# real-stanford/flingbot

Hardware: AMD Instinct MI355X
Metric: sim steps/sec (64x64-particle cloth) (higher is better)
Workload: dtype f32

## Files before the change

flingbot_amd/csrc/fs_fused_grid_kernel.h:

```cpp
#pragma once
#include "fs_fused_kernel.h"

#define FG_PLANE (FS_FUSED_MAX_PARTICLES * 4)
#define FG_PAD 1024
#define FG_OFF_XX FG_PAD
#define FG_OFF_X0 (FG_OFF_XX + 4 * FG_PLANE)
#define FG_OFF_CACC (FG_OFF_X0 + 3 * FG_PLANE)
#define FG_OFF_CUR (FG_OFF_CACC + FS_FUSED_CSET_CAP * 16)
#define FG_OFF_ITEMS (FG_OFF_CUR + FS_FUSED_CUR_BYTES)
#define FG_OFF_SCAN (FG_OFF_ITEMS + FS_FUSED_MAX_PARTICLES * 2)
#define FG_OFF_CSET (FG_OFF_SCAN + 64)
#define FG_OFF_CHIST (FG_OFF_CSET + FS_FUSED_CSET_CAP * 2)
#define FG_OFF_ROWL (FG_OFF_CHIST + 512)
#define FG_OFF_KZ (FG_OFF_ROWL + 1024)
#define FG_OFF_KS (FG_OFF_KZ + 1024)
#define FG_OFF_COLL (FG_OFF_KS + 1024)
#define FG_OFF_RCNT (FG_OFF_COLL + 512)
#define FG_LDS_BYTES (FG_OFF_RCNT + 512)
static_assert(FG_OFF_ROWL % 8 == 0 && (FG_OFF_KZ - FG_OFF_ROWL) % 8 == 0, "row tables are read as ds_read_b64 pairs");
static_assert((FG_OFF_COLL - FG_OFF_KS) % 256 == 0, "column tables share one address, rows as ds_read2st64_b32 offsets");
static_assert(FG_LDS_BYTES <= 160 * 1024, "grid-64 kernel: the LDS of one CU");
static_assert(FG_OFF_CACC % 16 == 0 && FG_OFF_CUR == FG_OFF_CACC + FS_FUSED_CSET_CAP * 16, "set and queue accumulators: one array");
#ifndef FG_SINGLES
#define FG_SINGLES 1
// ... 12 lines not shown
    asm volatile("ds_read2st64_b32 %0, %1 offset0:%2 offset1:%3" : "=v"(x0) : "v"(a), "n"(DZ + 2), "n"(DZ + 3) : "memory");
    asm volatile("ds_read2st64_b32 %0, %1 offset0:%2 offset1:%3" : "=v"(x1) : "v"(a), "n"(DZ + 2 + 64), "n"(DZ + 3 + 64) : "memory");
    asm volatile("ds_read2st64_b32 %0, %1 offset0:%2 offset1:%3" : "=v"(x2) : "v"(a), "n"(DZ + 2 + 128), "n"(DZ + 3 + 128) : "memory");
}
template <int OFF>
__device__ __forceinline__ fs_f2 fg_load_rows(unsigned a) {
    static_assert(OFF >= 0 && OFF < 65536 && OFF % 8 == 0, "ds_read_b64 offset");
    fs_f2 r;
    asm volatile("ds_read_b64 %0, %1 offset:%2" : "=v"(r) : "v"(a), "n"(OFF) : "memory");
    return r;
}
template <int R0, int R1>
__device__ __forceinline__ fs_f2 fg_load_cols(unsigned a) {
    static_assert(R0 >= 0 && R0 < 256 && R1 >= 0 && R1 < 256, "ds_read2st64_b32 offsets");
    fs_f2 r;
    asm volatile("ds_read2st64_b32 %0, %1 offset0:%2 offset1:%3" : "=v"(r) : "v"(a), "n"(R0), "n"(R1) : "memory");
    return r;
}
#define FG_WAIT(N, A0, A1, A2) asm volatile("s_waitcnt lgkmcnt(" #N ")" : "+v"(A0), "+v"(A1), "+v"(A2))

#define FG_MIN_L2 1.17549435e-38f
__device__ __forceinline__ float fg_scale(float xi0, float xi1, float xi2, float xj0, float xj1, float xj2, float L, float k,
                                          float &l2) {
    const float ex = xi0 - xj0, ey = xi1 - xj1, ez = xi2 - xj2;
    l2 = fs_dot3(ex, ey, ez, ex, ey, ez);
    const float inv = __builtin_amdgcn_rsqf(l2);
    const float len = l2 * inv;
    const float C = len - L;
    return k * (C * inv);
}
__device__ __forceinline__ void fg_accum(float &d0, float &d1, float &d2, float xi0, float xi1, float xi2, float xj0, float xj1,
                                         float xj2, float sc) {
    const float ex = xi0 - xj0, ey = xi1 - xj1, ez = xi2 - xj2;
    d0 = FS_FMA(-ex, sc, d0);
    d1 = FS_FMA(-ey, sc, d1);
    d2 = FS_FMA(-ez, sc, d2);
}
__device__ __forceinline__ float fg_from_left(float v) {
    return __int_as_float(__builtin_amdgcn_update_dpp(0, __float_as_int(v), 0x138, 0xf, 0xf, true));
}
__device__ __forceinline__ float fg_from_right(float v) {
    return __int_as_float(__builtin_amdgcn_update_dpp(0, __float_as_int(v), 0x130, 0xf, 0xf, true));
}

__device__ __forceinline__ void fg_apply(const FsAcc &a, float relax, const float *rcnt, float &x0, float &x1, float &x2) {
    if (a.cnt > 0) {
        const float sc = a.cnt < 128 ? rcnt[a.cnt] : relax / (float)a.cnt;
        x0 = FS_FMA(a.d0, sc, x0); x1 = FS_FMA(a.d1, sc, x1); x2 = FS_FMA(a.d2, sc, x2);
    }
}

__global__ __launch_bounds__(FS_FUSED_THREADS) void fs_k_fused_grid64(const FsEnvDev *__restrict__ envs,
                                                                      const FsShapesDev *__restrict__ shapes, const int *ids,
                                                                      int n_steps) {
    static_assert(FS_FUSED_THREADS == 1024 && FS_FUSED_PPT == 4, "grid-64 kernel: 16 waves x 4 rows");
    extern __shared__ __attribute__((aligned(16))) char smem[];
    float *Xx = (float *)(smem + FG_OFF_XX);
    float *Xy = Xx + FS_FUSED_MAX_PARTICLES, *Xz = Xy + FS_FUSED_MAX_PARTICLES, *Xw = Xz + FS_FUSED_MAX_PARTICLES;
    float *X0x = (float *)(smem + FG_OFF_X0);
    float *X0y = X0x + FS_FUSED_MAX_PARTICLES;
    float *X0z = X0y + FS_FUSED_MAX_PARTICLES;
    unsigned short *cursor = (unsigned short *)(smem + FG_OFF_CUR);
    unsigned short *items = (unsigned short *)(smem + FG_OFF_ITEMS);
    int *wave_tot = (int *)(smem + FG_OFF_SCAN);
    float *rowL = (float *)(smem + FG_OFF_ROWL);

#ifdef FS_BLOCK_CLOCKS
    const unsigned long long tc_start = __builtin_amdgcn_s_memtime(), tr_start = __builtin_amdgcn_s_memrealtime();
#endif
#ifdef FS_TIMING
    unsigned long long ts_acc[16] = {0, 0, 0, 0, 0, 0, 0, 0, 0, 0, 0, 0, 0, 0, 0, 0};
    unsigned long long ts_last = __builtin_amdgcn_s_memtime();
#endif
    const int e = ids[blockIdx.x];
    if (e < 0) return;
    const FsEnvDev &E = envs[e];
    const FsShapesDev &sh = shapes[e];
    const FsFusedConsts c = fs_fused_consts(E, sh);
    const int n = c.n;
    const unsigned un = (unsigned)n;
    const int t = threadIdx.x, lane = t & 63, w = t >> 6;
    const int dimz = n >> 6;

    FsVec4 *const g_pos = E.pos, *const g_vel = E.vel;
    const FsVec4 *const g_rest = E.rest;
    const fs_gci g_phase = (fs_gci)E.phase;
    const fs_gi g_nlist = (fs_gi)E.nlist, g_ncount = (fs_gi)E.ncount;
    const fs_gci g_ell_j = (fs_gci)E.ell_j;
    const fs_gcf g_ell_len = (fs_gcf)E.ell_len, g_ell_k = (fs_gcf)E.ell_k;
    const fs_gcf g_L = (fs_gcf)E.g64_L;
    const int max_deg = E.max_deg;
    const fs_gcu g_near = (fs_gcu)E.restnear_w;

    int find_mode = 0;
    {
        const int ph0 = g_phase[0];
        int differs = 0;
        for (int i = t; i < n; i += FS_FUSED_THREADS) differs |= (g_phase[i] != ph0);
        if (t == 0) wave_tot[0] = 0;
        __syncthreads();
        if (differs) atomicOr(&wave_tot[0], 1);
        __syncthreads();
        const int mixed = wave_tot[0];
        __syncthreads();
        if (!mixed) {
            if (!(ph0 & FS_PHASE_SELF_COLLIDE)) find_mode = 3;
            else if (!(ph0 & FS_PHASE_SELF_COLLIDE_FILTER)) find_mode = 2;
            else if (E.restnear_ok == 2 && FS_STENCIL_FILTER) find_mode = 4;
            else if (E.restnear_ok) find_mode = 1;
        }
    }
    for (int q = t; q < FG_OFF_X0 / 4; q += FS_FUSED_THREADS) ((float *)smem)[q] = 0.0f;
    __syncthreads();
    for (int i = t; i < n; i += FS_FUSED_THREADS) {
        const FsVec4 p = fs_ld4(g_pos, i);
        Xx[i] = p.x; Xy[i] = p.y; Xz[i] = p.z; Xw[i] = p.w;
        X0x[i] = p.x; X0y[i] = p.y; X0z[i] = p.z;
    }
    if (t < 256) {
        const int r = t & 63, s = 8 + (t >> 6);
        rowL[t] = r < dimz ? g_L[(unsigned)s * un + (unsigned)(r * 64 + 2)] : 0.0f;
    }
    constexpr int XS_DX[4] = {-1, -2, +1, +2};
    constexpr int SH_DX[4] = {+1, -1, -1, +1}, SH_DZ[4] = {-1, -1, +1, +1};
    constexpr int ZS_DZ[4] = {-1, -2, +1, +2};
    float *colL = (float *)(smem + FG_OFF_COLL);
    if (t < 128) {
        const int col = t & 63, q = t >> 6;
        const int dxq = q == 0 ? -1 : -2;
        colL[t] = (unsigned)(col + dxq) < 64u ? g_L[(unsigned)q * un + (unsigned)(2 * 64 + col)] : 0.0f;
    }
    float *rcnt = (float *)(smem + FG_OFF_RCNT);
    if (t < 128) rcnt[t] = t > 0 ? c.relax / (float)t : 0.0f;
    if (t < 256) {
        const int c64 = t & 63, q = t >> 6;
        const int sdx = (q == 0 || q == 3) ? +1 : -1, sslot = q < 2 ? 2 + q : 4 + q;
        const int zdz = q < 2 ? -1 - q : q - 1;
        ((float *)(smem + FG_OFF_KS))[t] = (unsigned)(c64 + sdx) < 64u ? E.g64_kh[sslot] : 0.0f;
        ((float *)(smem + FG_OFF_KZ))[t] = (c64 < dimz && (unsigned)(c64 + zdz) < (unsigned)dimz) ? E.g64_kh[8 + q] : 0.0f;
    }
    const float kh0 = E.g64_kh[0], kh1 = E.g64_kh[1];
    unsigned nvalid = 0u;
#pragma unroll
    for (int k = 0; k < FS_FUSED_PPT; ++k) {
        const int row = FG_ROW(w, k);
        int cnt = 0;
#pragma unroll
        for (int q = 0; q < 4; ++q) {
            cnt += ((unsigned)(lane + XS_DX[q]) < 64u) ? 1 : 0;
            cnt += ((unsigned)(lane + SH_DX[q]) < 64u && (unsigned)(row + SH_DZ[q]) < (unsigned)dimz) ? 1 : 0;
            cnt += ((unsigned)(row + ZS_DZ[q]) < (unsigned)dimz) ? 1 : 0;
        }
        nvalid |= (unsigned)cnt << (8 * k);
    }
    __syncthreads();
    unsigned fastmask = 0u;
    {
        constexpr int cdx[FS_G64_SLOTS] = FS_G64_DX_LIST, cdz[FS_G64_SLOTS] = FS_G64_DZ_LIST;
#pragma unroll
        for (int k = 0; k < FS_FUSED_PPT; ++k) {
            const int row = FG_ROW(w, k), i = row * 64 + lane;
            bool differs = false;
            if (i < n) {
                const float wi = Xw[i];
                differs = !(wi > 0.0f);
#pragma unroll
                for (int q = 0; q < FS_G64_SLOTS; ++q) {
                    const bool in = (unsigned)(lane + cdx[q]) < 64u && (unsigned)(row + cdz[q]) < (unsigned)dimz;
                    if (in) differs |= Xw[i + cdz[q] * 64 + cdx[q]] != wi;
                }
            }
            if (i < n && __builtin_amdgcn_ballot_w64(differs) == 0ull) fastmask |= 1u << k;
        }
        fastmask = (unsigned)__builtin_amdgcn_readfirstlane((int)fastmask);
    }

    FS_TS(0)
#pragma unroll 1
    for (int frame = 0; frame < n_steps; ++frame) {
#pragma unroll 1
        for (int sub = 0; sub < c.substeps; ++sub) {
            for (int q = t; q < FS_FUSED_BUCKETS / 2; q += FS_FUSED_THREADS) ((unsigned *)cursor)[q] = 0u;
            FsVec4 xp[FS_FUSED_PPT];
#pragma unroll
            for (int k = 0; k < FS_FUSED_PPT; ++k) {
                const int i = t + k * FS_FUSED_THREADS;
                xp[k] = FsVec4{0.0f, 0.0f, 0.0f, 0.0f};
                if (i < n) {
                    const FsVec4 p0 = FsVec4{X0x[i], X0y[i], X0z[i], Xw[i]};
                    xp[k] = fs_fused_predict(c, p0, fs_ld4(g_vel, i));
                    fs_st4(E.x0, i, p0);
                }
            }
            __syncthreads();
            const fs_lu fill = (fs_lu)(smem + FG_OFF_XX + 2 * FG_PLANE);
            if (find_mode == 4)
                for (int q = t; q < FS_FUSED_MAX_PARTICLES; q += FS_FUSED_THREADS) fill[q] = 0u;
            fs_fused_build_grid(c, xp, cursor, items, wave_tot, X0x, X0y, X0z);
            FS_TS(1)
            const FsFindConsts fc = {n, c.ncap, c.rad2, c.inv_rad, find_mode, E.gp_dimx, E.gp_magic};
            if (find_mode == 4) {
                int *const any_over = wave_tot;
                if (t == 0) *any_over = 0;
                int sb0 = 0, sb1 = 0, sb2 = 0, sb3 = 0;
#pragma unroll 1
                for (int k = 0; k < FS_FUSED_PPT; ++k) {
                    const int qs = t + k * FS_FUSED_THREADS;
                    if (qs >= n) break;
                    const int i = items[qs];
                    const FsVec4 xi = FsVec4{X0x[qs], X0y[qs], X0z[qs], 0.0f};
                    const int shape_bits = (int)(fs_shape_candidates(E.p, sh, sub, xi.x, xi.y, xi.z) << FS_SHAPE_MASK_SHIFT);
                    if (k == 0) sb0 = shape_bits; else if (k == 1) sb1 = shape_bits; else if (k == 2) sb2 = shape_bits; else sb3 = shape_bits;
                    fs_pair_find_neighbors(fc, i, qs, xi, (fs_lcus)cursor, (fs_lcus)items, g_nlist, (fs_lus)(smem + FG_OFF_XX) + t,
                                           (fs_lcf)X0x, fill);
                }
                FS_TS(2)
                __syncthreads();
                FS_TS(3)
                unsigned overmask = 0u;
#pragma unroll 1
                for (int k = 0; k < FS_FUSED_PPT; ++k) {
                    const int qs = t + k * FS_FUSED_THREADS;
                    if (qs >= n) break;
                    const int i = items[qs];
                    const int cnt = (int)fill[i];
                    const int shape_bits = k == 0 ? sb0 : k == 1 ? sb1 : k == 2 ? sb2 : sb3;
                    if (cnt > c.ncap) {
                        overmask |= 1u << k;
                        continue;
                    }
                    fs_pair_sort_column(n, i, cnt, g_nlist);
                    g_ncount[i] = cnt | shape_bits;
                }
                if (overmask) atomicOr(any_over, 1);
                __syncthreads();
                if (*any_over) {
                    FsNearWords none;
#pragma unroll
                    for (int q = 0; q < 8; ++q) none.w[q] = 0xffffffffu;
#pragma unroll 1
                    for (int k = 0; k < FS_FUSED_PPT; ++k) {
                        if (!((overmask >> k) & 1u)) continue;
                        const int qs = t + k * FS_FUSED_THREADS;
                        const int i = items[qs];
                        const FsVec4 xi = FsVec4{X0x[qs], X0y[qs], X0z[qs], 0.0f};
                        const int shape_bits = k == 0 ? sb0 : k == 1 ? sb1 : k == 2 ? sb2 : sb3;
                        g_ncount[i] = fs_fused_find_neighbors<true>(fc, i, xi, (fs_lcus)cursor, (fs_lcus)items, g_phase, g_rest, g_nlist,
                                                                    none, (fs_lus)(smem + FG_OFF_XX) + t, (fs_lcf)X0x) | shape_bits;
                    }
                    __syncthreads();
                }
            } else {
#pragma unroll 1
                for (int qs = t; qs < n; qs += FS_FUSED_THREADS) {
                    const int i = items[qs];
                    const FsVec4 xi = FsVec4{X0x[qs], X0y[qs], X0z[qs], 0.0f};
                    const int shape_bits = (int)(fs_shape_candidates(E.p, sh, sub, xi.x, xi.y, xi.z) << FS_SHAPE_MASK_SHIFT);
                    FsNearWords near;
#pragma unroll
                    for (int q = 0; q < 8; ++q) near.w[q] = find_mode == 1 ? g_near[(unsigned)q * un + (unsigned)i] : 0xffffffffu;
                    g_ncount[i] = (find_mode == 3 ? 0
                                                  : fs_fused_find_neighbors<false>(fc, i, xi, (fs_lcus)cursor, (fs_lcus)items, g_phase,
                                                                                   g_rest, g_nlist, near,
                                                                                   (fs_lus)(smem + FG_OFF_XX) + t, (fs_lcf)X0x)) |
                                  shape_bits;
                }
                FS_TS(2)
                __syncthreads();
                FS_TS(3)
            }
#pragma unroll
            for (int k = 0; k < FS_FUSED_PPT; ++k) {
                const int i = t + k * FS_FUSED_THREADS;
                if (i < n) {
                    Xx[i] = xp[k].x; Xy[i] = xp[k].y; Xz[i] = xp[k].z; Xw[i] = xp[k].w;
                    const FsVec4 p0 = fs_ld4(E.x0, i);
                    X0x[i] = p0.x; X0y[i] = p0.y; X0z[i] = p0.z;
                } else {
                    Xx[i] = 0.0f; Xy[i] = 0.0f; Xz[i] = 0.0f; Xw[i] = 0.0f;
                }
            }

            unsigned short *cset = (unsigned short *)(smem + FG_OFF_CSET);
            FsVec4 *cacc = (FsVec4 *)(smem + FG_OFF_CACC);
            int *chist = (int *)(smem + FG_OFF_CHIST);
            if (t < 128) chist[t] = 0;
            int *nsingles = (int *)(smem + FG_OFF_SCAN);
            if (t == 0) *nsingles = 0;
            __syncthreads();
            int ccls[FS_FUSED_PPT];
#pragma unroll
            for (int k = 0; k < FS_FUSED_PPT; ++k) {
                const int i = FG_ROW(w, k) * 64 + lane;
                int cc = 0;
                if (i < n && Xw[i] > 0.0f) cc = g_ncount[i] & FS_NCOUNT_MASK;
                ccls[k] = cc > 96 ? 96 : cc;
                if (ccls[k] > 0) atomicAdd(&chist[ccls[k]], 1);
            }
            __syncthreads();
            fs_fused_count_offsets(chist, t);
            __syncthreads();
            FsVec4 *squeue = cacc + FS_FUSED_CSET_CAP;
            unsigned slotw[2] = {~0u, ~0u};
#pragma unroll
            for (int k = 0; k < FS_FUSED_PPT; ++k) {
                if (ccls[k] > 0) {
                    const int i = FG_ROW(w, k) * 64 + lane;
                    unsigned slot = FG_SLOT_INLINE;
                    const int pos = atomicAdd(&chist[ccls[k]], 1);
                    if (pos < FS_FUSED_CSET_CAP) {
                        cset[pos] = (unsigned short)i;
                        slot = (unsigned)pos;
                    }
#if FG_SINGLES
                    else if (ccls[k] <= 16) {
                        const int sp = atomicAdd(nsingles, 1);
                        if (sp < FG_SINGLES_CAP) {
                            slot = (unsigned)(FS_FUSED_CSET_CAP + sp);
                            squeue[sp].w = __int_as_float(i | (g_nlist[i] << 12) | ((ccls[k] - 1) << 28));
                        }
                    }
#endif
                    slotw[k >> 1] = (slotw[k >> 1] & ~(0xffffu << (16 * (k & 1)))) | (slot << (16 * (k & 1)));
                }
            }
            __syncthreads();
            const int csize = chist[0] < FS_FUSED_CSET_CAP ? chist[0] : FS_FUSED_CSET_CAP;
            const int n_singles = *nsingles < FG_SINGLES_CAP ? *nsingles : FG_SINGLES_CAP;
            const int i2 = t < csize ? (int)cset[t] : -1;
            int cnt2 = 0, cj2[FS_FUSED_PREFETCH_CAND];
#pragma unroll
            for (int q = 0; q < FS_FUSED_PREFETCH_CAND; ++q) cj2[q] = 0;
            if (i2 >= 0) {
                cnt2 = g_ncount[i2] & FS_NCOUNT_MASK;
#pragma unroll
                for (int q = 0; q < FS_FUSED_PREFETCH_CAND; ++q) cj2[q] = g_nlist[(unsigned)q * un + (unsigned)i2];
            }
            static_assert(FG_SINGLES_CAP <= 2 * FG_SINGLES_LANES, "two queue entries per lane");
            unsigned qw0 = 0u, qw1 = 0u;
#if FG_SINGLES
            if (t >= 64 && t - 64 < n_singles) qw0 = (unsigned)__float_as_int(squeue[t - 64].w);
            if (t >= 64 && t - 64 + FG_SINGLES_LANES < n_singles) qw1 = (unsigned)__float_as_int(squeue[t - 64 + FG_SINGLES_LANES].w);
            __syncthreads();
#endif

            FS_TS(4)
#pragma unroll 1
            for (int it = 0; it < c.iters; ++it) {
                unsigned cpack = 0u;
                float rold[2][3], rnew[2][3];
#pragma unroll
                for (int q = 0; q < 6; ++q) { rold[q / 3][q % 3] = 0.0f; rnew[q / 3][q % 3] = 0.0f; }
#ifdef FG_UNROLL_PAIRS
#pragma unroll
#else
#pragma unroll 1
#endif
                for (int pr = 0; pr < 2; ++pr) {
                    const int rowP = FG_ROW(w, 2 * pr);
                    const int iP_raw = rowP * 64 + lane, iQ_raw = iP_raw + 64;
                    const bool haveP = rowP < dimz, haveQ = rowP + 1 < dimz;
                    const int iP = haveP ? iP_raw : 0, iQ = haveQ ? iQ_raw : 0;
                    const bool fast = haveQ && ((fastmask >> (2 * pr)) & 3u) == 3u;
                    const fs_f2 xi0 = fs_f2{Xx[iP], Xx[iQ]}, xi1 = fs_f2{Xy[iP], Xy[iQ]}, xi2 = fs_f2{Xz[iP], Xz[iQ]};
                    const fs_f2 wi = fs_f2{Xw[iP], Xw[iQ]};
                    FsAcc aP, aQ;
                    bool exact = !fast;
                    if (fast) {
                        unsigned aLane = (unsigned)(lane * 4);
                        asm volatile("" : "+v"(aLane));
                        const unsigned am2 = (unsigned)(FG_OFF_XX + ((rowP - 2) * 64 - 2) * 4) + aLane;
                        const unsigned am1 = am2 + 4u, a00 = am2 + 8u, ap1 = am2 + 12u, ap2 = am2 + 16u;
                        constexpr int SH_SLOT[4] = {2, 3, 6, 7};
                        float sLP[2], sLQ[4];
#pragma unroll
                        for (int q = 0; q < 2; ++q) sLP[q] = g_L[(unsigned)SH_SLOT[q] * un + (unsigned)iP];
#pragma unroll
                        for (int q = 0; q < 4; ++q) sLQ[q] = g_L[(unsigned)SH_SLOT[q] * un + (unsigned)iQ];
                        const unsigned aRow = (unsigned)(FG_OFF_ROWL + rowP * 4), aCol = (unsigned)FG_OFF_KS + aLane;
                        constexpr int CL_ROW = (FG_OFF_COLL - FG_OFF_KS) / 256;
                        fs_f2 cL = fg_load_cols<CL_ROW, CL_ROW + 1>(aCol);
                        const unsigned aKP = rowP >= 1 ? aCol : aLane;
                        const unsigned aKQ = rowP + 2 < dimz ? aCol : aLane;
                        fs_f2 kP23 = fg_load_cols<0, 1>(aKP);
                        fs_f2 kQ23 = fg_load_cols<0, 1>(aCol);
#define FG_KX(q) ((unsigned)(lane + XS_DX[q]) < 64u ? (q == 0 ? kh0 : kh1) : 0.0f)
                        float dP0 = 0.0f, dP1 = 0.0f, dP2 = 0.0f, dQ0 = 0.0f, dQ1 = 0.0f, dQ2 = 0.0f, mP = 1.0f, mQ = 1.0f;
                        fs_f2 u0, u1, u2, v0, v1, v2;
                        float l2a, l2b, l2c, l2d;
                        fg_load_slot<0>(am1, u0, u1, u2);
                        fg_load_slot<0>(am2, v0, v1, v2);
                        asm volatile("s_waitcnt lgkmcnt(3)"
                                     : "+v"(cL), "+v"(kP23), "+v"(kQ23), "+v"(u0), "+v"(u1), "+v"(u2));
                        const float scP0 = fg_scale(xi0.x, xi1.x, xi2.x, u0.x, u1.x, u2.x, cL.x, FG_KX(0), l2a);
                        const float scQ0 = fg_scale(xi0.y, xi1.y, xi2.y, u0.y, u1.y, u2.y, cL.x, FG_KX(0), l2b);
                        fg_accum(dP0, dP1, dP2, xi0.x, xi1.x, xi2.x, u0.x, u1.x, u2.x, scP0);
                        fg_accum(dQ0, dQ1, dQ2, xi0.y, xi1.y, xi2.y, u0.y, u1.y, u2.y, scQ0);
                        __builtin_amdgcn_sched_barrier(0);
                        fg_load_slot<-1>(ap1, u0, u1, u2);
                        FG_WAIT(3, v0, v1, v2);
                        const float scP1 = fg_scale(xi0.x, xi1.x, xi2.x, v0.x, v1.x, v2.x, cL.y, FG_KX(1), l2c);
                        const float scQ1 = fg_scale(xi0.y, xi1.y, xi2.y, v0.y, v1.y, v2.y, cL.y, FG_KX(1), l2d);
                        fg_accum(dP0, dP1, dP2, xi0.x, xi1.x, xi2.x, v0.x, v1.x, v2.x, scP1);
                        fg_accum(dQ0, dQ1, dQ2, xi0.y, xi1.y, xi2.y, v0.y, v1.y, v2.y, scQ1);
                        mP = fminf(fminf(mP, l2a), l2c);
                        mQ = fminf(fminf(mQ, l2b), l2d);
                        __builtin_amdgcn_sched_barrier(0);
                        fg_load_slot<-1>(am1, v0, v1, v2);
// ... 191 lines not shown
                    int jn = more > 0 ? g_nlist[un + (unsigned)i] : 0;
                    const FsVec4 pa = squeue[q];
                    FsAcc a = {pa.x, pa.y, pa.z, __float_as_int(pa.w)};
                    const float xi0 = Xx[i], xi1 = Xy[i], xi2 = Xz[i], wi = Xw[i];
                    const float ri0 = xi0 - X0x[i], ri1 = xi1 - X0y[i], ri2 = xi2 - X0z[i];
#pragma unroll 1
                    for (int sq = 0; sq <= more; ++sq) {
                        const FsVec4 xj = FsVec4{Xx[j], Xy[j], Xz[j], Xw[j]};
                        fs_particle_contact(a, xi0, xi1, xi2, wi, ri0, ri1, ri2, xj, xj.x - X0x[j], xj.y - X0y[j], xj.z - X0z[j], c.restd,
                                            c.restd2, c.mu_p);
                        j = jn;
                        if (sq + 2 <= more) jn = g_nlist[(unsigned)(sq + 2) * un + (unsigned)i];
                    }
                    squeue[q] = FsVec4{a.d0, a.d1, a.d2, __int_as_float(a.cnt)};
                }
#endif
                FS_TS(8)
                __syncthreads();
                FS_TS(9)
#pragma unroll 1
                for (int pr = 0; pr < 2; ++pr) {
                    const int iP = FG_ROW(w, 2 * pr) * 64 + lane;
                    const unsigned slw = pr == 0 ? slotw[0] : slotw[1];
                    FsAcc a[2];
                    unsigned sm[2];
                    bool act[2];
                    float x0[2], x1[2], x2[2], r0[2], r1[2], r2[2];
                    int n_planes = c.n_planes, n_shapes = c.n_shapes;
                    asm volatile("" : "+s"(n_planes), "+s"(n_shapes));
#pragma unroll
                    for (int h = 0; h < 2; ++h) {
                        const int i = iP + 64 * h;
                        const unsigned myslot = h == 0 ? (slw & 0xffffu) : (slw >> 16);
                        act[h] = (i < n) & (Xw[i] > 0.0f);
                        a[h] = FsAcc{rold[h][0], rold[h][1], rold[h][2], (int)(h == 0 ? cpack >> 24 : (cpack >> 16) & 0xffu)};
                        if (act[h] && myslot < FG_SLOT_INLINE) {
                            const FsVec4 pa = cacc[myslot];
                            a[h] = FsAcc{pa.x, pa.y, pa.z, __float_as_int(pa.w)};
                        }
                        sm[h] = act[h] ? (pr == 0 ? smk[h] : smk[2 + h]) : 0u;
                        x0[h] = Xx[i]; x1[h] = Xy[i]; x2[h] = Xz[i];
                        r0[h] = x0[h] - X0x[i]; r1[h] = x1[h] - X0y[i]; r2[h] = x2[h] - X0z[i];
                    }
#pragma unroll
                    for (int q = 0; q < 3; ++q) { rold[0][q] = rnew[0][q]; rold[1][q] = rnew[1][q]; }
                    cpack <<= 16;
#pragma unroll
                    for (int h = 0; h < 2; ++h) {
                        int q = 0;
                        if (n_planes == 1) {
                            if (sm[h] & 1u)
                                fs_plane_contact(a[h], x0[h], x1[h], x2[h], r0[h], r1[h], r2[h], c.pl0, c.pl1, c.pl2, c.pl3, c.cd, c.mu_s,
                                                 c.mu_k);
                            q = 1;
                        }
                        for (; q < n_planes; ++q)
                            if ((sm[h] >> q) & 1u)
                                fs_plane_contact(a[h], x0[h], x1[h], x2[h], r0[h], r1[h], r2[h], E.p.planes[q][0], E.p.planes[q][1],
                                                 E.p.planes[q][2], E.p.planes[q][3], c.cd, c.mu_s, c.mu_k);
                    }
                    if (n_shapes != 0 && __builtin_amdgcn_ballot_w64(((sm[0] | sm[1]) >> FS_SHAPE_SPHERE_BIT) != 0u) != 0ull) {
                        const float S = (float)c.substeps;
#pragma unroll
                        for (int h = 0; h < 2; ++h)
                            for (int q = 0; q < n_shapes; ++q)
                                if ((sm[h] >> (FS_SHAPE_SPHERE_BIT + q)) & 1u) {
                                    float c0, c1, c2, s0, s1, s2;
                                    fs_shape_sweep(sh, q, sub, S, c0, c1, c2, s0, s1, s2);
                                    fs_sphere_contact(a[h], x0[h], x1[h], x2[h], r0[h], r1[h], r2[h], c0, c1, c2, sh.pos[q].w, s0, s1, s2,
                                                      c.cd, c.mu_s, c.mu_k);
                                }
                    }
#pragma unroll
                    for (int h = 0; h < 2; ++h)
                        if (act[h]) {
                            const int i = iP + 64 * h;
                            fg_apply(a[h], c.relax, rcnt, x0[h], x1[h], x2[h]);
                            Xx[i] = x0[h]; Xy[i] = x1[h]; Xz[i] = x2[h];
                        }
                }
                __syncthreads();
                FS_TS(10)
            }
            for (int i = t; i < n; i += FS_FUSED_THREADS) {
                const FsVec4 xf = FsVec4{Xx[i], Xy[i], Xz[i], Xw[i]};
                FsVec4 p0 = FsVec4{X0x[i], X0y[i], X0z[i], xf.w};
                FsVec4 v = fs_ld4(g_vel, i);
                fs_fused_finalize(c, p0, v, xf);
                fs_st4(g_vel, i, v);
                X0x[i] = p0.x; X0y[i] = p0.y; X0z[i] = p0.z;
            }
        }
    }
    for (int i = t; i < n; i += FS_FUSED_THREADS) fs_st4(g_pos, i, FsVec4{X0x[i], X0y[i], X0z[i], Xw[i]});
#ifdef FS_BLOCK_CLOCKS
    if (t == 0) {
        const unsigned long long tc_total = __builtin_amdgcn_s_memtime() - tc_start, tr_end = __builtin_amdgcn_s_memrealtime();
        const fs_gi out = g_nlist + 95u * un;
        out[0] = (int)(unsigned)tc_total; out[1] = (int)(unsigned)(tc_total >> 32);
        out[2] = (int)(unsigned)tr_start; out[3] = (int)(unsigned)tr_end;
    }
#endif
#ifdef FS_TIMING
    FS_TS(11)
#ifdef FS_TIMING_COUNTS
    if (blockIdx.x == 0 && t == 0)
        printf("DBG runs(wave) %llu trips(wave) %llu candidates(lane) %llu survivors(lane) %llu accepted(lane) %llu phaseB trips(wave) %llu\n",
               fs_dbg_cnt[0], fs_dbg_cnt[1], fs_dbg_cnt[2], fs_dbg_cnt[3], fs_dbg_cnt[4], fs_dbg_cnt[5]);
#endif
    if (blockIdx.x == 0 && (t & 63) == 0)
        printf("TS wave %2d: init %llu grid %llu find %llu findwait %llu cset %llu springs %llu park %llu bar1 %llu contact %llu bar2 %llu finish+bar3 %llu final %llu\n",
               t >> 6, ts_acc[0], ts_acc[1], ts_acc[2], ts_acc[3], ts_acc[4], ts_acc[5], ts_acc[6], ts_acc[7], ts_acc[8], ts_acc[9], ts_acc[10],
               ts_acc[11]);
#endif
}
```

flingbot_amd/csrc/fs_fused_kernel.h:

```cpp
#pragma once
#include "fs_constraints.h"
#include "fs_pair_search.h"

#ifndef FS_FUSED_THREADS
#define FS_FUSED_THREADS 1024
#endif
#define FS_FUSED_PPT (4096 / FS_FUSED_THREADS)
#define FS_FUSED_MAX_PARTICLES (FS_FUSED_THREADS * FS_FUSED_PPT)
#define FS_FUSED_MAX_DEG 64
#ifndef FS_STENCIL_FILTER
#define FS_STENCIL_FILTER 1
#endif
#ifndef FS_FUSED_BUCKET_BITS
#define FS_FUSED_BUCKET_BITS 13
#endif
#define FS_FUSED_BUCKETS (1 << FS_FUSED_BUCKET_BITS)
#define FS_FUSED_CUR_BYTES (FS_FUSED_BUCKETS * 2)
#define FS_FUSED_SLOTS 16

#define FS_FUSED_OFF_DICT 0
#define FS_FUSED_OFF_X (FS_FUSED_OFF_DICT + 256 * 8)
#define FS_FUSED_OFF_X0 (FS_FUSED_OFF_X + FS_FUSED_MAX_PARTICLES * 16)
#define FS_FUSED_OFF_CUR (FS_FUSED_OFF_X0 + FS_FUSED_MAX_PARTICLES * 12)
#define FS_FUSED_OFF_ITEMS (FS_FUSED_OFF_CUR + FS_FUSED_CUR_BYTES)
// ... 39 lines not shown
__device__ __forceinline__ void fs_st4o(FsVec4 *base, unsigned idx, const FsVec4 v) {
    *(FS_GLOBAL fs_f4 *)((FS_GLOBAL char *)base + (idx << 4)) = fs_f4{v.x, v.y, v.z, v.w};
}
template <typename T>
__device__ __forceinline__ T fs_ldo(const T *base, unsigned idx) {
    return *(FS_GLOBAL const T *)((FS_GLOBAL const char *)base + (idx << 2));
}

__device__ __forceinline__ int fs_fused_row(int cy, int cz) {
    return fs_pair_row(cy, cz, FS_FUSED_BUCKET_BITS);
}
__device__ __forceinline__ int fs_fused_bucket(int cx, int cy, int cz) {
    return (fs_fused_row(cy, cz) + cx) & (FS_FUSED_BUCKETS - 1);
}

struct FsFusedConsts {
    int n, substeps, iters, ncap, n_shapes, n_planes;
    float h, inv_h, g0, g1, g2, damping;
    float rad2, inv_rad, restd, restd2, mu_p, mu_s, mu_k, cd, relax, maxdv2, maxdv, thr2, max_speed;
    float pl0, pl1, pl2, pl3;
};

__device__ __forceinline__ FsFusedConsts fs_fused_consts(const FsEnvDev &E, const FsShapesDev &sh) {
    const FsParams &p = E.p;
    FsFusedConsts c;
    c.n = E.n; c.substeps = p.numSubsteps; c.iters = p.numIterations;
    c.ncap = p.maxNeighbors < FS_MAX_NEIGHBORS ? p.maxNeighbors : FS_MAX_NEIGHBORS;
    c.n_shapes = sh.count; c.n_planes = p.numPlanes;
    c.h = p.dt / (float)p.numSubsteps;
    c.inv_h = 1.0f / c.h;
    c.g0 = p.gravity[0]; c.g1 = p.gravity[1]; c.g2 = p.gravity[2]; c.damping = p.damping;
    const float rad = p.radius + p.particleCollisionMargin;
    c.rad2 = rad * rad; c.inv_rad = 1.0f / rad;
    c.restd = p.solidRestDistance; c.restd2 = c.restd * c.restd;
    c.mu_p = p.particleFriction; c.mu_s = p.staticFriction; c.mu_k = p.dynamicFriction;
    c.cd = p.collisionDistance; c.relax = p.relaxationFactor;
    c.maxdv = p.maxAcceleration * c.h; c.maxdv2 = c.maxdv * c.maxdv;
    c.thr2 = p.sleepThreshold * p.sleepThreshold; c.max_speed = p.maxSpeed;
    c.pl0 = p.planes[0][0]; c.pl1 = p.planes[0][1]; c.pl2 = p.planes[0][2]; c.pl3 = p.planes[0][3];
    return c;
}

__device__ __forceinline__ FsVec4 fs_fused_predict(const FsFusedConsts &c, const FsVec4 pos, const FsVec4 vel) {
    FsVec4 xp = pos;
    if (pos.w > 0.0f) {
        float vx = vel.x + c.h * (c.g0 - c.damping * vel.x);
        float vy = vel.y + c.h * (c.g1 - c.damping * vel.y);
        float vz = vel.z + c.h * (c.g2 - c.damping * vel.z);
        xp.x = pos.x + c.h * vx;
        xp.y = pos.y + c.h * vy;
        xp.z = pos.z + c.h * vz;
    }
    return xp;
}

__device__ __forceinline__ void fs_fused_finalize(const FsFusedConsts &c, FsVec4 &pos, FsVec4 &vel, const FsVec4 xp) {
    if (!(pos.w > 0.0f)) {
        vel = FsVec4{0.0f, 0.0f, 0.0f, 0.0f};
        return;
    }
    float vx = (xp.x - pos.x) * c.inv_h, vy = (xp.y - pos.y) * c.inv_h, vz = (xp.z - pos.z) * c.inv_h;
    float ax = vx - vel.x, ay = vy - vel.y, az = vz - vel.z;
    float dv2 = ax * ax + ay * ay + az * az;
    if (dv2 > c.maxdv2) {
        float sc = c.maxdv / sqrtf(dv2);
        vx = vel.x + ax * sc; vy = vel.y + ay * sc; vz = vel.z + az * sc;
    }
    float v2 = vx * vx + vy * vy + vz * vz;
    if (c.max_speed < 3.402823466e+38f && v2 > c.max_speed * c.max_speed) {
        float sc = c.max_speed / sqrtf(v2);
        vx = vx * sc; vy = vy * sc; vz = vz * sc;
        v2 = vx * vx + vy * vy + vz * vz;
    }
    if (v2 < c.thr2) {
        vel = FsVec4{0.0f, 0.0f, 0.0f, 0.0f};
    } else {
        vel = FsVec4{vx, vy, vz, 0.0f};
        pos.x = xp.x; pos.y = xp.y; pos.z = xp.z;
    }
}

__device__ __forceinline__ void fs_fused_build_grid(const FsFusedConsts &c, const FsVec4 (&xp)[FS_FUSED_PPT],
                                                    unsigned short *cursor, unsigned short *items, int *wave_tot, float *XSx,
                                                    float *XSy, float *XSz) {
    const int t = threadIdx.x, lane = t & 63, wave = t >> 6;
    unsigned *cw = (unsigned *)cursor;
    int bucket[FS_FUSED_PPT];
#pragma unroll
    for (int k = 0; k < FS_FUSED_PPT; ++k) {
        const int i = t + k * FS_FUSED_THREADS;
        bucket[k] = fs_fused_bucket((int)floorf(xp[k].x * c.inv_rad), (int)floorf(xp[k].y * c.inv_rad),
                                    (int)floorf(xp[k].z * c.inv_rad));
        if (i < c.n) atomicAdd(&cw[bucket[k] >> 1], 1u << ((bucket[k] & 1) << 4));
    }
    __syncthreads();
    {
        constexpr int PW = FS_FUSED_BUCKETS / FS_FUSED_THREADS / 2;
        static_assert(PW >= 1 && PW * 2 * FS_FUSED_THREADS == FS_FUSED_BUCKETS, "bucket table: whole words per thread");
        unsigned wv[PW];
        int sum = 0;
#pragma unroll
        for (int k = 0; k < PW; ++k) { wv[k] = cw[t * PW + k]; sum += (int)(wv[k] & 0xffffu) + (int)(wv[k] >> 16); }
        int inc = sum;
        for (int off = 1; off < 64; off <<= 1) {
            int o = __shfl_up(inc, off, 64);
            if (lane >= off) inc += o;
        }
        if (lane == 63) wave_tot[wave] = inc;
        __syncthreads();
        int run = inc - sum;
        for (int w = 0; w < wave; ++w) run += wave_tot[w];
#pragma unroll
        for (int k = 0; k < PW; ++k) {
            const unsigned lo = (unsigned)run;
            run += (int)(wv[k] & 0xffffu);
            const unsigned hi = (unsigned)run;
            run += (int)(wv[k] >> 16);
            cw[t * PW + k] = lo | (hi << 16);
        }
    }
    __syncthreads();
#pragma unroll
    for (int k = 0; k < FS_FUSED_PPT; ++k) {
        const int i = t + k * FS_FUSED_THREADS;
        if (i < c.n) {
            const unsigned sh = (unsigned)(bucket[k] & 1) << 4;
            const int slot = (int)((atomicAdd(&cw[bucket[k] >> 1], 1u << sh) >> sh) & 0xffffu);
            items[slot] = (unsigned short)i;
            XSx[slot] = xp[k].x; XSy[slot] = xp[k].y; XSz[slot] = xp[k].z;
        }
    }
    __syncthreads();
}

struct FsFindConsts {
    int n, ncap;
    float rad2, inv_rad;
    int mode;
    int dimx;
    unsigned magic;
};
struct FsNearWords {
    uint32_t w[8];
};
 #ifdef FS_TIMING
__device__ unsigned long long fs_dbg_cnt[8];
#define FS_DBG_COUNT(k, v)                                                                                   \
    if (blockIdx.x == 0) {                                                                                   \
        const int l_ = threadIdx.x & 63;                                                                     \
        if (__builtin_amdgcn_readfirstlane(l_) == l_) atomicAdd(&fs_dbg_cnt[k], (unsigned long long)(v));   \
    }
#define FS_DBG_LANE(k, v) \
    if (blockIdx.x == 0) atomicAdd(&fs_dbg_cnt[k], (unsigned long long)(v));
#else
#define FS_DBG_COUNT(k, v)
#define FS_DBG_LANE(k, v)
#endif
#ifdef FS_TIMING_COUNTS
#define FS_CNT_WAVE(k, v) FS_DBG_COUNT(k, v)
#define FS_CNT_LANE(k, v) FS_DBG_LANE(k, v)
#else
#define FS_CNT_WAVE(k, v)
#define FS_CNT_LANE(k, v)
#endif
#define FS_FUSED_FINDQ 32

#define FS_NB_EMPTY 0x7fffffff
#ifndef FS_NB_STAGED_FUSED
#define FS_NB_STAGED_FUSED 4
#endif
#ifndef FS_NB_STAGED_STREAM
#define FS_NB_STAGED_STREAM 8
#endif
template <int ST>
struct FsNbListT {
    int a[ST];
    int gcnt;
};
template <int ST>
__device__ __forceinline__ FsNbListT<ST> fs_nb_empty() {
    FsNbListT<ST> L;
#pragma unroll
    for (int q = 0; q < ST; ++q) L.a[q] = FS_NB_EMPTY;
    L.gcnt = 0;
    return L;
}

template <int ST>
__device__ __forceinline__ void fs_fused_global_insert(int n, int i, int j, int gcap, int &gcnt, fs_gi nlist) {
    if (gcap <= 0) return;
    fs_gi list = nlist + (size_t)ST * n + i;
    int s = gcnt, prev = -1;
    while (s > 0) {
        prev = list[(size_t)(s - 1) * n];
        if (prev <= j) break;
        --s;
    }
    if (s > 0 && prev == j) return;
    if (gcnt == gcap) {
        if (s == gcap) return;
        gcnt = gcap - 1;
    }
    for (int u = gcnt; u > s; --u) list[(size_t)u * n] = list[(size_t)(u - 1) * n];
    list[(size_t)s * n] = j;
    ++gcnt;
}

template <bool STENCIL = false, int ST = FS_NB_STAGED_STREAM>
__device__ __forceinline__ void fs_fused_accept(const FsFindConsts &c, int i, int j, FsNbListT<ST> &L, int &phi, FsVec4 &ri,
                                                bool &have_meta, fs_gci phase, const FsVec4 *rest, fs_gi nlist,
                                                const FsNearWords &near) {
    if (STENCIL) {
// ... 364 lines not shown
    const fs_gi g_nlist = (fs_gi)E.nlist, g_ncount = (fs_gi)E.ncount;
    const fs_gci g_ell_j = (fs_gci)E.ell_j;
    const fs_gcf g_ell_len = (fs_gcf)E.ell_len, g_ell_k = (fs_gcf)E.ell_k;
    const fs_gcu g_nbr = (fs_gcu)E.nbr_w, g_code = (fs_gcu)E.code_w;
    const int max_deg = E.max_deg;

    float2 dict_e = make_float2(0.0f, 0.0f);
    bool dict_bad = false;
    if (COMPACT && t < 256) {
        const fs_gcf g_dict = (fs_gcf)E.dict;
        dict_e = make_float2(g_dict[2 * t], g_dict[2 * t + 1]);
        dict_bad = t < E.dict_size && (dict_e.y < 0.0f || (dict_e.y * 0.5f) * 2.0f != dict_e.y);
    }
    const fs_gcu g_near = (fs_gcu)E.restnear_w;
    int find_mode = 0;
    bool dict_halved = false;
    {
        const int ph0 = g_phase[0];
        int differs = 0;
        for (int i = t; i < n; i += FS_FUSED_THREADS) differs |= (g_phase[i] != ph0);
        if (t == 0) { wave_tot[0] = 0; wave_tot[1] = 0; }
        __syncthreads();
        if (differs) atomicOr(&wave_tot[0], 1);
        if (dict_bad) atomicOr(&wave_tot[1], 1);
        __syncthreads();
        const int mixed = wave_tot[0];
        dict_halved = COMPACT && wave_tot[1] == 0;
        __syncthreads();
        if (!mixed) {
            if (!(ph0 & FS_PHASE_SELF_COLLIDE)) find_mode = 3;
            else if (!(ph0 & FS_PHASE_SELF_COLLIDE_FILTER)) find_mode = 2;
            else if (E.restnear_ok == 2 && FS_STENCIL_FILTER) find_mode = 4;
            else if (E.restnear_ok) find_mode = 1;
        }
    }
    if (COMPACT && t < 256)
        *(float2 *)(smem + FS_FUSED_OFF_DICT + t * 8) = make_float2(dict_e.x, dict_halved ? dict_e.y * 0.5f : dict_e.y);
    const float kscale = dict_halved ? 2.0f : 1.0f;
    for (int i = t; i < n; i += FS_FUSED_THREADS) {
        const FsVec4 p = fs_ld4(g_pos, i);
        X[i] = p;
        X0x[i] = p.x; X0y[i] = p.y; X0z[i] = p.z;
    }
    unsigned fastmask = 0u;
    if (COMPACT && dict_halved) {
        __syncthreads();
#pragma unroll
        for (int k = 0; k < FS_FUSED_PPT; ++k) {
            const int i = t + k * FS_FUSED_THREADS;
            bool differs = false;
            if (i < n) {
                const float wi = X[i].w;
                if (wi > 0.0f) {
#pragma unroll
                    for (int q = 0; q < JW; ++q) {
                        const uint32_t w = g_nbr[(unsigned)q * un + (unsigned)i];
                        differs |= *(const float *)(smem + FS_FUSED_OFF_X + (w & 0xffffu) + 12) != wi;
                        differs |= *(const float *)(smem + FS_FUSED_OFF_X + (w >> 16) + 12) != wi;
                    }
                }
            }
            if (__builtin_amdgcn_ballot_w64(differs) == 0ull) fastmask |= 1u << k;
        }
    }

    FS_TS(0)
#pragma unroll 1
    for (int frame = 0; frame < n_steps; ++frame) {
#pragma unroll 1
        for (int sub = 0; sub < c.substeps; ++sub) {
            for (int q = t; q < FS_FUSED_BUCKETS / 2; q += FS_FUSED_THREADS) ((unsigned *)cursor)[q] = 0u;
            FsVec4 xp[FS_FUSED_PPT];
#pragma unroll
            for (int k = 0; k < FS_FUSED_PPT; ++k) {
                const int i = t + k * FS_FUSED_THREADS;
                xp[k] = FsVec4{0.0f, 0.0f, 0.0f, 0.0f};
                if (i < n) {
                    const FsVec4 p0 = FsVec4{X0x[i], X0y[i], X0z[i], X[i].w};
                    xp[k] = fs_fused_predict(c, p0, fs_ld4(g_vel, i));
                    fs_st4(E.x0, i, p0);
                }
            }
            __syncthreads();
            fs_fused_build_grid(c, xp, cursor, items, wave_tot, X0x, X0y, X0z);
            FS_TS(1)
            const FsFindConsts fc = {n, c.ncap, c.rad2, c.inv_rad, find_mode, E.gp_dimx, E.gp_magic};
#pragma unroll 1
            for (int qs = t; qs < n; qs += FS_FUSED_THREADS) {
                const int i = items[qs];
                const FsVec4 xi = FsVec4{X0x[qs], X0y[qs], X0z[qs], 0.0f};
                const int shape_bits = (int)(fs_shape_candidates(E.p, sh, sub, xi.x, xi.y, xi.z) << FS_SHAPE_MASK_SHIFT);
                if (find_mode == 4) {
                    FsNearWords none;
#pragma unroll
                    for (int q = 0; q < 8; ++q) none.w[q] = 0xffffffffu;
                    g_ncount[i] = fs_fused_find_neighbors<true>(fc, i, xi, (fs_lcus)cursor, (fs_lcus)items, g_phase, g_rest, g_nlist,
                                                                none, (fs_lus)(smem + FS_FUSED_OFF_X) + t, (fs_lcf)X0x) | shape_bits;
                    continue;
                }
                FsNearWords near;
#pragma unroll
                for (int q = 0; q < 8; ++q) near.w[q] = find_mode == 1 ? g_near[(unsigned)q * un + (unsigned)i] : 0xffffffffu;
                g_ncount[i] = (find_mode == 3 ? 0
                                              : fs_fused_find_neighbors<false>(fc, i, xi, (fs_lcus)cursor, (fs_lcus)items, g_phase,
                                                                               g_rest, g_nlist, near,
                                                                               (fs_lus)(smem + FS_FUSED_OFF_X) + t, (fs_lcf)X0x)) |
                              shape_bits;
            }
            FS_TS(2)
            __syncthreads();
            FS_TS(3)
#pragma unroll
            for (int k = 0; k < FS_FUSED_PPT; ++k) {
                const int i = t + k * FS_FUSED_THREADS;
                if (i < n) {
                    X[i] = xp[k];
                    const FsVec4 p0 = fs_ld4(E.x0, i);
                    X0x[i] = p0.x; X0y[i] = p0.y; X0z[i] = p0.z;
                }
            }

            unsigned short *cset = (unsigned short *)(smem + FS_FUSED_OFF_CSET);
            FsVec4 *cacc = (FsVec4 *)(smem + FS_FUSED_OFF_CACC);
            int *chist = (int *)(smem + FS_FUSED_OFF_CHIST);
            if (t < 128) chist[t] = 0;
            int *nqueued = (int *)(smem + FS_FUSED_OFF_SCAN);
            if (t == 0) *nqueued = 0;
            __syncthreads();
            int ccls[FS_FUSED_PPT];
#pragma unroll
            for (int k = 0; k < FS_FUSED_PPT; ++k) {
                const int i = t + k * FS_FUSED_THREADS;
                int cc = 0;
                if (i < n && X[i].w > 0.0f) cc = g_ncount[i] & FS_NCOUNT_MASK;
                ccls[k] = cc > 96 ? 96 : cc;
                if (ccls[k] > 0) atomicAdd(&chist[ccls[k]], 1);
            }
            __syncthreads();
            fs_fused_count_offsets(chist, t);
            __syncthreads();
            unsigned long long slotpack[(FS_FUSED_PPT + 3) / 4];
#pragma unroll
            for (int q = 0; q < (FS_FUSED_PPT + 3) / 4; ++q) slotpack[q] = ~0ull;
#pragma unroll
            for (int k = 0; k < FS_FUSED_PPT; ++k) {
                if (ccls[k] > 0) {
                    const int pos = atomicAdd(&chist[ccls[k]], 1);
                    if (pos < FS_FUSED_CSET_CAP) {
                        cset[pos] = (unsigned short)(t + k * FS_FUSED_THREADS);
                        slotpack[k >> 2] = (slotpack[k >> 2] & ~(0xffffull << (16 * (k & 3)))) |
                                           ((unsigned long long)pos << (16 * (k & 3)));
                    }
#if FS_FUSED_QUEUE
                    else if (ccls[k] <= 8) {
                        const int sp = atomicAdd(nqueued, 1);
                        if (sp < FS_FUSED_QUEUE_CAP)
                            slotpack[k >> 2] = (slotpack[k >> 2] & ~(0xffffull << (16 * (k & 3)))) |
                                               ((unsigned long long)(FS_FUSED_CSET_CAP + sp) << (16 * (k & 3)));
                    }
#endif
                }
            }
            __syncthreads();
            const int csize = chist[0] < FS_FUSED_CSET_CAP ? chist[0] : FS_FUSED_CSET_CAP;
            const int n_queued = *nqueued < FS_FUSED_QUEUE_CAP ? *nqueued : FS_FUSED_QUEUE_CAP;
            FsVec4 *squeue = (FsVec4 *)(smem + FS_FUSED_OFF_CUR);
            const int i2 = t < csize ? (int)cset[t] : -1;
// ... 221 lines not shown
```

Baseline: 142,400.

## Keep particle state in registers across substeps and reuse grid slots

Position and velocity are now held in per-thread registers across substeps, so predict no longer reloads velocity from global memory and the final position store comes from registers. After the grid sort, each thread records its sorted slot and reads the predicted position back from the sorted LDS arrays instead of keeping xp live. Neighbour counts are prefetched into registers before the contact-set build. asm volatile barriers pin loop indices and constants to VGPRs so the compiler cannot rematerialize them. The cost is more register pressure and extra code paths, plus new timing probes.

```diff
diff --git a/flingbot_amd/csrc/fs_fused_grid_kernel.h b/flingbot_amd/csrc/fs_fused_grid_kernel.h
--- a/flingbot_amd/csrc/fs_fused_grid_kernel.h
+++ b/flingbot_amd/csrc/fs_fused_grid_kernel.h
@@ -118,7 +118,7 @@
     const int t = threadIdx.x, lane = t & 63, w = t >> 6;
     const int dimz = n >> 6;
 
-    FsVec4 *const g_pos = E.pos, *const g_vel = E.vel;
+    FsVec4 *const g_pos = E.pos;
     const FsVec4 *const g_rest = E.rest;
     const fs_gci g_phase = (fs_gci)E.phase;
     const fs_gi g_nlist = (fs_gi)E.nlist, g_ncount = (fs_gi)E.ncount;
@@ -211,28 +211,57 @@
         fastmask = (unsigned)__builtin_amdgcn_readfirstlane((int)fastmask);
     }
 
+    FsVec4 sx[FS_FUSED_PPT], sv[FS_FUSED_PPT];
+#pragma unroll
+    for (int k = 0; k < FS_FUSED_PPT; ++k) {
+        const int i = t + k * FS_FUSED_THREADS;
+        sx[k] = FsVec4{0.0f, 0.0f, 0.0f, 0.0f};
+        sv[k] = FsVec4{0.0f, 0.0f, 0.0f, 0.0f};
+        if (i < n) {
+            sv[k] = fs_ld4o(E.vel, (unsigned)i);
+            sx[k] = FsVec4{X0x[i], X0y[i], X0z[i], Xw[i]};
+        }
+    }
+
     FS_TS(0)
 #pragma unroll 1
     for (int frame = 0; frame < n_steps; ++frame) {
 #pragma unroll 1
         for (int sub = 0; sub < c.substeps; ++sub) {
-            for (int q = t; q < FS_FUSED_BUCKETS / 2; q += FS_FUSED_THREADS) ((unsigned *)cursor)[q] = 0u;
             FsVec4 xp[FS_FUSED_PPT];
-#pragma unroll
-            for (int k = 0; k < FS_FUSED_PPT; ++k) {
-                const int i = t + k * FS_FUSED_THREADS;
-                xp[k] = FsVec4{0.0f, 0.0f, 0.0f, 0.0f};
-                if (i < n) {
-                    const FsVec4 p0 = FsVec4{X0x[i], X0y[i], X0z[i], Xw[i]};
-                    xp[k] = fs_fused_predict(c, p0, fs_ld4(g_vel, i));
-                    fs_st4(E.x0, i, p0);
-                }
-            }
+            {
+                unsigned tl = (unsigned)t;
+                asm volatile("" : "+v"(tl));
+                for (unsigned q = tl; q < FS_FUSED_BUCKETS / 2; q += FS_FUSED_THREADS) ((unsigned *)cursor)[q] = 0u;
+                FsFusedConsts cf = c;
+                asm volatile("" : "+v"(cf.h), "+v"(cf.g0), "+v"(cf.g1), "+v"(cf.g2), "+v"(cf.damping));
+#pragma unroll
+                for (int k = 0; k < FS_FUSED_PPT; ++k) {
+                    const unsigned i = tl + (unsigned)(k * FS_FUSED_THREADS);
+                    xp[k] = FsVec4{0.0f, 0.0f, 0.0f, 0.0f};
+                    if (i < un) xp[k] = fs_fused_predict(cf, sx[k], sv[k]);
+                }
+#pragma unroll
+                for (int k = 0; k < FS_FUSED_PPT; ++k) {
+                    const unsigned i = tl + (unsigned)(k * FS_FUSED_THREADS);
+                    if (i < un) fs_st4o(E.x0, i, sx[k]);
+                }
+            }
+            FS_TS(12)
             __syncthreads();
             const fs_lu fill = (fs_lu)(smem + FG_OFF_XX + 2 * FG_PLANE);
-            if (find_mode == 4)
-                for (int q = t; q < FS_FUSED_MAX_PARTICLES; q += FS_FUSED_THREADS) fill[q] = 0u;
-            fs_fused_build_grid(c, xp, cursor, items, wave_tot, X0x, X0y, X0z);
+            if (find_mode == 4) {
+                unsigned tl = (unsigned)t;
+                asm volatile("" : "+v"(tl));
+                for (unsigned q = tl; q < FS_FUSED_MAX_PARTICLES; q += FS_FUSED_THREADS) fill[q] = 0u;
+            }
+            unsigned xslot[2];
+            {
+                int slot_of[FS_FUSED_PPT] = {0, 0, 0, 0};
+                fs_fused_build_grid(c, xp, cursor, items, wave_tot, X0x, X0y, X0z, slot_of);
+                xslot[0] = (unsigned)slot_of[0] | ((unsigned)slot_of[1] << 16);
+                xslot[1] = (unsigned)slot_of[2] | ((unsigned)slot_of[3] << 16);
+            }
             FS_TS(1)
             const FsFindConsts fc = {n, c.ncap, c.rad2, c.inv_rad, find_mode, E.gp_dimx, E.gp_magic};
             if (find_mode == 4) {
@@ -286,6 +315,7 @@
                     }
                     __syncthreads();
                 }
+                FS_TS(15)
             } else {
 #pragma unroll 1
                 for (int qs = t; qs < n; qs += FS_FUSED_THREADS) {
@@ -305,18 +335,36 @@
                 __syncthreads();
                 FS_TS(3)
             }
-#pragma unroll
-            for (int k = 0; k < FS_FUSED_PPT; ++k) {
-                const int i = t + k * FS_FUSED_THREADS;
-                if (i < n) {
-                    Xx[i] = xp[k].x; Xy[i] = xp[k].y; Xz[i] = xp[k].z; Xw[i] = xp[k].w;
-                    const FsVec4 p0 = fs_ld4(E.x0, i);
-                    X0x[i] = p0.x; X0y[i] = p0.y; X0z[i] = p0.z;
-                } else {
-                    Xx[i] = 0.0f; Xy[i] = 0.0f; Xz[i] = 0.0f; Xw[i] = 0.0f;
-                }
-            }
-
+            FsVec4 p0r[FS_FUSED_PPT];
+            int cword[FS_FUSED_PPT];
+            {
+                unsigned tl = (unsigned)t;
+                asm volatile("" : "+v"(tl));
+#pragma unroll
+                for (int k = 0; k < FS_FUSED_PPT; ++k) {
+                    const unsigned i = tl + (unsigned)(k * FS_FUSED_THREADS);
+                    p0r[k] = fs_ld4o(E.x0, i < un ? i : 0u);
+                }
+                const unsigned wl = tl >> 6, ll = tl & 63u;
+#pragma unroll
+                for (int k = 0; k < FS_FUSED_PPT; ++k) {
+                    const unsigned i = (unsigned)FG_ROW(wl, k) * 64u + ll;
+                    cword[k] = fs_ldo((const int *)E.ncount, i < un ? i : 0u);
+                }
+#pragma unroll
+                for (int k = 0; k < FS_FUSED_PPT; ++k) {
+                    const unsigned i = tl + (unsigned)(k * FS_FUSED_THREADS);
+                    const unsigned s = (xslot[k >> 1] >> (16 * (k & 1))) & 0xffffu;
+                    const float x = X0x[s], y = X0y[s], z = X0z[s];
+                    if (i < un) {
+                        Xx[i] = x; Xy[i] = y; Xz[i] = z; Xw[i] = p0r[k].w;
+                    } else {
+                        Xx[i] = 0.0f; Xy[i] = 0.0f; Xz[i] = 0.0f; Xw[i] = 0.0f;
+                    }
+                }
+            }
+
+            FS_TS(13)
             unsigned short *cset = (unsigned short *)(smem + FG_OFF_CSET);
             FsVec4 *cacc = (FsVec4 *)(smem + FG_OFF_CACC);
             int *chist = (int *)(smem + FG_OFF_CHIST);
@@ -324,12 +372,24 @@
             int *nsingles = (int *)(smem + FG_OFF_SCAN);
             if (t == 0) *nsingles = 0;
             __syncthreads();
+            {
+                unsigned tl = (unsigned)t;
+                asm volatile("" : "+v"(tl));
+#pragma unroll
+                for (int k = 0; k < FS_FUSED_PPT; ++k) {
+                    const unsigned i = tl + (unsigned)(k * FS_FUSED_THREADS);
+                    if (i < un) { X0x[i] = p0r[k].x; X0y[i] = p0r[k].y; X0z[i] = p0r[k].z; }
+                }
+            }
+            unsigned tq = (unsigned)t;
+            asm volatile("" : "+v"(tq));
+            const int wq = (int)(tq >> 6), lq = (int)(tq & 63u);
             int ccls[FS_FUSED_PPT];
 #pragma unroll
             for (int k = 0; k < FS_FUSED_PPT; ++k) {
-                const int i = FG_ROW(w, k) * 64 + lane;
+                const int i = FG_ROW(wq, k) * 64 + lq;
                 int cc = 0;
-                if (i < n && Xw[i] > 0.0f) cc = g_ncount[i] & FS_NCOUNT_MASK;
+                if (i < n && Xw[i] > 0.0f) cc = cword[k] & FS_NCOUNT_MASK;
                 ccls[k] = cc > 96 ? 96 : cc;
                 if (ccls[k] > 0) atomicAdd(&chist[ccls[k]], 1);
             }
@@ -341,7 +401,7 @@
 #pragma unroll
             for (int k = 0; k < FS_FUSED_PPT; ++k) {
                 if (ccls[k] > 0) {
-                    const int i = FG_ROW(w, k) * 64 + lane;
+                    const int i = FG_ROW(wq, k) * 64 + lq;
                     unsigned slot = FG_SLOT_INLINE;
                     const int pos = atomicAdd(&chist[ccls[k]], 1);
                     if (pos < FS_FUSED_CSET_CAP) {
@@ -353,13 +413,14 @@
                         const int sp = atomicAdd(nsingles, 1);
                         if (sp < FG_SINGLES_CAP) {
                             slot = (unsigned)(FS_FUSED_CSET_CAP + sp);
-                            squeue[sp].w = __int_as_float(i | (g_nlist[i] << 12) | ((ccls[k] - 1) << 28));
+                            squeue[sp].w = __int_as_float(i | (fs_ldo((const int *)E.nlist, (unsigned)i) << 12) | ((ccls[k] - 1) << 28));
                         }
                     }
 #endif
                     slotw[k >> 1] = (slotw[k >> 1] & ~(0xffffu << (16 * (k & 1)))) | (slot << (16 * (k & 1)));
                 }
             }
+            FS_TS(14)
             __syncthreads();
             const int csize = chist[0] < FS_FUSED_CSET_CAP ? chist[0] : FS_FUSED_CSET_CAP;
             const int n_singles = *nsingles < FG_SINGLES_CAP ? *nsingles : FG_SINGLES_CAP;
@@ -717,17 +778,36 @@
                 __syncthreads();
                 FS_TS(10)
             }
-            for (int i = t; i < n; i += FS_FUSED_THREADS) {
-                const FsVec4 xf = FsVec4{Xx[i], Xy[i], Xz[i], Xw[i]};
-                FsVec4 p0 = FsVec4{X0x[i], X0y[i], X0z[i], xf.w};
-                FsVec4 v = fs_ld4(g_vel, i);
-                fs_fused_finalize(c, p0, v, xf);
-                fs_st4(g_vel, i, v);
-                X0x[i] = p0.x; X0y[i] = p0.y; X0z[i] = p0.z;
+            {
+                unsigned tl = (unsigned)t;
+                asm volatile("" : "+v"(tl));
+#pragma unroll
+                for (int k = 0; k < FS_FUSED_PPT; ++k) {
+                    const unsigned i = tl + (unsigned)(k * FS_FUSED_THREADS);
+                    sv[k] = fs_ld4o(E.vel, i < un ? i : 0u);
+                }
+                FsFusedConsts cf = c;
+                asm volatile("" : "+v"(cf.inv_h), "+v"(cf.maxdv2), "+v"(cf.maxdv), "+v"(cf.max_speed), "+v"(cf.thr2));
+#pragma unroll
+                for (int k = 0; k < FS_FUSED_PPT; ++k) {
+                    const unsigned i = tl + (unsigned)(k * FS_FUSED_THREADS);
+                    const FsVec4 xf = FsVec4{Xx[i], Xy[i], Xz[i], Xw[i]};
+                    sx[k] = FsVec4{X0x[i], X0y[i], X0z[i], xf.w};
+                    fs_fused_finalize(cf, sx[k], sv[k], xf);
+                }
+#pragma unroll
+                for (int k = 0; k < FS_FUSED_PPT; ++k) {
+                    const unsigned i = tl + (unsigned)(k * FS_FUSED_THREADS);
+                    if (i < un) fs_st4o(E.vel, i, sv[k]);
+                }
             }
         }
     }
-    for (int i = t; i < n; i += FS_FUSED_THREADS) fs_st4(g_pos, i, FsVec4{X0x[i], X0y[i], X0z[i], Xw[i]});
+#pragma unroll
+    for (int k = 0; k < FS_FUSED_PPT; ++k) {
+        const int i = t + k * FS_FUSED_THREADS;
+        if (i < n) fs_st4o(g_pos, (unsigned)i, sx[k]);
+    }
 #ifdef FS_BLOCK_CLOCKS
     if (t == 0) {
         const unsigned long long tc_total = __builtin_amdgcn_s_memtime() - tc_start, tr_end = __builtin_amdgcn_s_memrealtime();
@@ -744,8 +824,8 @@
                fs_dbg_cnt[0], fs_dbg_cnt[1], fs_dbg_cnt[2], fs_dbg_cnt[3], fs_dbg_cnt[4], fs_dbg_cnt[5]);
 #endif
     if (blockIdx.x == 0 && (t & 63) == 0)
-        printf("TS wave %2d: init %llu grid %llu find %llu findwait %llu cset %llu springs %llu park %llu bar1 %llu contact %llu bar2 %llu finish+bar3 %llu final %llu\n",
-               t >> 6, ts_acc[0], ts_acc[1], ts_acc[2], ts_acc[3], ts_acc[4], ts_acc[5], ts_acc[6], ts_acc[7], ts_acc[8], ts_acc[9], ts_acc[10],
-               ts_acc[11]);
+        printf("TS wave %2d: init %llu predict %llu grid %llu find %llu findwait %llu sort %llu restore %llu alloc %llu cset %llu springs %llu park %llu bar1 %llu contact %llu bar2 %llu finish+bar3 %llu final %llu\n",
+               t >> 6, ts_acc[0], ts_acc[12], ts_acc[1], ts_acc[2], ts_acc[3], ts_acc[15], ts_acc[13], ts_acc[14], ts_acc[4], ts_acc[5], ts_acc[6],
+               ts_acc[7], ts_acc[8], ts_acc[9], ts_acc[10], ts_acc[11]);
 #endif
 }
diff --git a/flingbot_amd/csrc/fs_fused_kernel.h b/flingbot_amd/csrc/fs_fused_kernel.h
--- a/flingbot_amd/csrc/fs_fused_kernel.h
+++ b/flingbot_amd/csrc/fs_fused_kernel.h
@@ -145,7 +145,7 @@
 
 __device__ __forceinline__ void fs_fused_build_grid(const FsFusedConsts &c, const FsVec4 (&xp)[FS_FUSED_PPT],
                                                     unsigned short *cursor, unsigned short *items, int *wave_tot, float *XSx,
-                                                    float *XSy, float *XSz) {
+                                                    float *XSy, float *XSz, int (&slot_of)[FS_FUSED_PPT]) {
     const int t = threadIdx.x, lane = t & 63, wave = t >> 6;
     unsigned *cw = (unsigned *)cursor;
     int bucket[FS_FUSED_PPT];
@@ -191,6 +191,7 @@
             const int slot = (int)((atomicAdd(&cw[bucket[k] >> 1], 1u << sh) >> sh) & 0xffffu);
             items[slot] = (unsigned short)i;
             XSx[slot] = xp[k].x; XSy[slot] = xp[k].y; XSz[slot] = xp[k].z;
+            slot_of[k] = slot;
         }
     }
     __syncthreads();
@@ -721,7 +722,8 @@
                 }
             }
             __syncthreads();
-            fs_fused_build_grid(c, xp, cursor, items, wave_tot, X0x, X0y, X0z);
+            int slot_unused[FS_FUSED_PPT];
+            fs_fused_build_grid(c, xp, cursor, items, wave_tot, X0x, X0y, X0z, slot_unused);
             FS_TS(1)
             const FsFindConsts fc = {n, c.ncap, c.rad2, c.inv_rad, find_mode, E.gp_dimx, E.gp_magic};
 #pragma unroll 1
```

Result: faster. 147,600 (median of 6 runs) (+3.7%).
